# idonahum/photoVerse

Measured on AMD Instinct MI355X. Metric: denoising steps/sec at 512x512 bs=16, 50-step loop (2 UNet fwd + CFG + DPM-Solver++ step per step), higher is better.
Workload: dtype f16; 1 GPU; configs[1] shape timed over 96 steps instead of 50: SD-v1.5 UNet + PhotoVerse processors, 96-step loop, bs=16/GPU, 512x512 (64x64 latents), P=1, guidance 7.5, fp16; per_gpu_batch=16, global_batch=16, latent=64, parallelism=dp1 (batch-sharded, 1 all_gather), hip_graph=True, graph_branches=2

## Files before the change

### photoverse_amd/csrc/pv_gemm.hip

```cpp
#include "pv_gemm_dev.h"

namespace {

constexpr int BK = 64;
constexpr int ROW_BYTES = BK * 2;

template <int NF, int MIV = 4>
struct TileCfg {
    static constexpr int MI = MIV;
    static constexpr int BM = 2 * MI * 16;
    static constexpr int BN = NF * 32;
    static constexpr int NWAVES = 4;
    static constexpr int THREADS = NWAVES * 64;
    static constexpr int A_PER_WAVE = BM / 8 / NWAVES;
    static constexpr int STAGES = 2;
    static constexpr int A_BYTES = BM * ROW_BYTES;
    static constexpr int B_BYTES = BN * ROW_BYTES;
    static constexpr int STAGE_BYTES = A_BYTES + B_BYTES;
    static constexpr int SMEM_BYTES = STAGES * STAGE_BYTES;
    static constexpr int B_PIECES = NF * 4;
    static constexpr int B_PER_WAVE = (B_PIECES + NWAVES - 1) / NWAVES;
};

__device__ __forceinline__ float epi_act(float x, int act) {
    if (act == PV_ACT_SILU) return pv_silu(x);
    if (act == PV_ACT_QUICK_GELU) return pv_quick_gelu(x);
    if (act == PV_ACT_LEAKY_RELU) return x > 0.f ? x : 0.01f * x;
    return x;
}

__device__ __forceinline__ half8_t lds_frag(const char* base, int row, int chunk) {
    return *reinterpret_cast<const half8_t*>(base + row * ROW_BYTES + ((chunk ^ (row & 7)) << 4));
}

template <int N>
__device__ __forceinline__ void wait_vmcnt() {
    static_assert(N >= 0 && N < 64, "vmcnt is a 6-bit field");
    asm volatile("s_waitcnt vmcnt(%0)" ::"n"(N) : "memory");
}


__device__ __forceinline__ float row16_sum(float v) {
    v += __builtin_bit_cast(float, __builtin_amdgcn_update_dpp(0, __builtin_bit_cast(int, v), 0x128, 0xf, 0xf, false));
    v += __builtin_bit_cast(float, __builtin_amdgcn_update_dpp(0, __builtin_bit_cast(int, v), 0x124, 0xf, 0xf, false));
    v += __builtin_bit_cast(float, __builtin_amdgcn_update_dpp(0, __builtin_bit_cast(int, v), 0x122, 0xf, 0xf, false));
    v += __builtin_bit_cast(float, __builtin_amdgcn_update_dpp(0, __builtin_bit_cast(int, v), 0x121, 0xf, 0xf, false));
    return v;
}

template <int NF, bool CONV, bool GEGLU, bool CS = false, bool MULTI = false, int MIV = 4>
__global__ __launch_bounds__(256, MIV == 4 ? 2 : 3) void gemm_conv_kernel(const pv_gemm_params_dev p, const int tiles_n,
                                                                              const int nblk, const int order, const int tpw_arg) {
    const int tpw = MULTI ? tpw_arg : 1;
    using Cfg = TileCfg<NF, MIV>;
    static_assert(MIV == 4 || (!CS && !MULTI && !CONV), "the 64-row tile exists for plain Linear layers only");
    constexpr int BM = Cfg::BM;
    constexpr int NW = Cfg::NWAVES;
    constexpr int MI = Cfg::MI;
    constexpr int AP = Cfg::A_PER_WAVE;
    extern __shared__ __attribute__((aligned(16))) char smem[];

    const int lane = pv_lane_id();
    const int wave = pv_wave_id();
    const int bid = (order & 2) ? (int)blockIdx.x : pv_xcd_remap((int)blockIdx.x, nblk);
    const int m_fast = order & 1;
    const int tiles_m = nblk / tiles_n;
    const int tile_m = m_fast ? bid % tiles_m : bid / tiles_n;
    const int tile_n = (m_fast ? bid / tiles_m : bid % tiles_n) * tpw;
    const int m0 = tile_m * BM;
    int n0 = tile_n * Cfg::BN;

    const int cin = p.c0 + p.c1;
    const int K = p.taps * cin;
    const int nk_total = K / BK;
    const int nk_per = (nk_total + (int)gridDim.y - 1) / (int)gridDim.y;
    const int k_begin = (int)blockIdx.y * nk_per;
    const int nk = max(0, min(nk_total, k_begin + nk_per) - k_begin);

    const int lrow = lane >> 3;
    const int src_chunk = (lane & 7) ^ lrow;
    const int lane_cc2 = src_chunk * 16;
// ... 445 lines not shown
    if ((int)strlen(probe.name) >= name_len) return (int)hipErrorInvalidValue;
    strcpy(name, probe.name);
    if (workgroups) *workgroups = probe.wgs;
    return 0;
}

extern "C" int pv_gemm_conv(const pv_gemm_params* pp, void* stream_) {
    pv_gemm_params_dev p;
    static_cast<pv_gemm_params&>(p) = *pp;
    hipStream_t stream = reinterpret_cast<hipStream_t>(stream_);
    const int cin = p.c0 + p.c1;
    if (p.M <= 0 || p.N <= 0 || cin <= 0 || (cin % 64) || (p.c0 % 64) || (p.taps != 1 && p.taps != 9) || p.act == PV_ACT_GELU || p.splitk < 0 || p.splitk > 16 ||
        !p.a0 || !p.w || !p.out || (p.c1 && !p.a1) || p.hout * p.wout <= 0)
        return (int)hipErrorInvalidValue;
    if (p.colstats && (p.geglu || p.out_f32)) return (int)hipErrorInvalidValue;
    if (p.taps == 9 && !(p.pad == 1 || (p.pad == 0 && p.stride == 2 && !p.upsample))) return (int)hipErrorInvalidValue;
    {
        const size_t a_rows = p.taps == 9 ? (size_t)p.batch * p.hin * p.win : (size_t)p.M;
        const size_t b0 = ((a_rows - 1) * p.lda0 + p.c0) * 2, b1 = p.c1 ? ((a_rows - 1) * p.lda1 + p.c1) * 2 : 0;
        const size_t bw = (size_t)p.N * p.taps * cin * 2;
        if (b0 >= (1ull << 31) || b1 >= (1ull << 31) || bw >= (1ull << 31)) return (int)hipErrorInvalidValue;
        p.a0_bytes = (uint32_t)b0;
        p.a1_bytes = (uint32_t)b1;
        p.w_bytes = (uint32_t)bw;
    }
    if (p.geglu && (p.taps != 1 || (p.N % 128))) return (int)hipErrorInvalidValue;
    if (p.a_norm && (p.taps != 9 || (p.a_norm_act != PV_ACT_NONE && p.a_norm_act != PV_ACT_SILU))) return (int)hipErrorInvalidValue;
    {
        const int rc = pv_conv_big_launch(p, stream);
        if (rc >= 0) return rc;
        if (rc == -2 || p.a_norm) return (int)hipErrorInvalidValue;
    }
    if (p.ln_rowsum) return (int)hipErrorInvalidValue;
    if (p.geglu) return dispatch<4, false, true>(p, stream);
    const bool conv = p.taps == 9;
    if (p.N % 160 == 0) return conv ? dispatch<5, true, false>(p, stream) : dispatch<5, false, false>(p, stream);
    if (p.N % 128 == 0) return conv ? dispatch<4, true, false>(p, stream) : dispatch<4, false, false>(p, stream);
    return (int)hipErrorInvalidValue;
}
```

### photoverse_amd/csrc/pv_gemm_dev.h

```cpp
#pragma once
#include "pv_common.h"

struct pv_gemm_params_dev : pv_gemm_params {
    uint32_t a0_bytes, a1_bytes, w_bytes;
};

__attribute__((visibility("hidden"))) int pv_conv_big_launch(const pv_gemm_params_dev& p, hipStream_t stream);


__attribute__((visibility("hidden"))) int pv_gemm_splitk_reduce_launch(const pv_gemm_params_dev& p, int splits, hipStream_t stream);


struct pv_launch_probe {
    char name[160];
    long wgs;
};
extern thread_local pv_launch_probe* pv_gemm_probe;
```

### photoverse_amd/csrc/pv_rowgemm.hip

```cpp
#include "pv_common.h"
#include <stdlib.h>

namespace {

constexpr int RG_K = 320;
constexpr int RG_CHUNK = 160;
constexpr int RG_TILE = RG_CHUNK * 128;
constexpr int RG_SLOTS = 4;
constexpr int RG_SMEM = RG_SLOTS * RG_TILE;

struct pv_rowgemm_params_dev : pv_row_gemm_params {
    uint32_t w_bytes;
};

template <int N>
__device__ __forceinline__ void rg_wait_vmcnt() {
    static_assert(N >= 0 && N < 64, "vmcnt is a 6-bit field");
    asm volatile("s_waitcnt vmcnt(%0)" ::"n"(N) : "memory");
}

template <bool GEGLU>
__global__ __launch_bounds__(256, 2) void row_gemm_kernel(const pv_rowgemm_params_dev p) {
    constexpr int C = RG_K;
    constexpr int KK = C / 32;
    constexpr int KT = C / 64;
    constexpr int NFC = RG_CHUNK / 16;
    typedef unsigned uint4_t __attribute__((ext_vector_type(4)));
    typedef unsigned uint2_t __attribute__((ext_vector_type(2)));
    extern __shared__ __attribute__((aligned(16))) char smem[];

    const int lane = pv_lane_id(), wave = pv_wave_id();
    const int fr = lane & 15, g = lane >> 4;
    const int m0 = (int)blockIdx.x * 128;
    const int rows_here = min(128, p.M - m0);
    const int n_chunks = p.N / RG_CHUNK;
    const int NT = n_chunks * KT;

    const __amdgpu_buffer_rsrc_t rw = __builtin_amdgcn_make_buffer_rsrc(const_cast<void*>(p.w), 0, (int)p.w_bytes, 0x00020000);
    const __amdgpu_buffer_rsrc_t rx = __builtin_amdgcn_make_buffer_rsrc(const_cast<half_t*>(reinterpret_cast<const half_t*>(p.x)) + (size_t)m0 * p.ld_x, 0,
                                                                        rows_here * p.ld_x * 2, 0x00020000);
    const int ld_o = p.ld_out;
    const __amdgpu_buffer_rsrc_t ro = __builtin_amdgcn_make_buffer_rsrc(reinterpret_cast<half_t*>(p.out) + (size_t)m0 * ld_o, 0, rows_here * ld_o * 2, 0x00020000);

    const int lrow = lane >> 3;
    const unsigned w_lane_off = (unsigned)lrow * (unsigned)(C * 2) + (unsigned)(((lane & 7) ^ lrow) << 4);
    const unsigned piece_off = w_lane_off + (unsigned)(wave * 8) * (unsigned)(C * 2);
    auto issue_stage = [&](int t) {
        const int nc = t / KT, kt = t - nc * KT;
        char* dst = smem + (t & (RG_SLOTS - 1)) * RG_TILE;
        const int soff = nc * RG_CHUNK * (C * 2) + kt * 128;
#pragma unroll
        for (int i = 0; i < 5; ++i)
            __builtin_amdgcn_raw_ptr_buffer_load_lds(rw, PV_LDS_PTR(dst + (wave + 4 * i) * 1024), 16, (int)piece_off, soff + i * 32 * (C * 2), 0, 0);
    };
    auto wg_barrier = [&]() {
        asm volatile("s_waitcnt lgkmcnt(0)" ::: "memory");
        __builtin_amdgcn_s_barrier();
        asm volatile("" ::: "memory");
    };

    half8_t xf[KK][2];
    int mrow[2];
#pragma unroll
    for (int qi = 0; qi < 2; ++qi) {
        mrow[qi] = wave * 32 + qi * 16 + fr;
        const int off = mrow[qi] * p.ld_x * 2 + g * 16;
#pragma unroll
        for (int kk = 0; kk < KK; ++kk) xf[kk][qi] = __builtin_bit_cast(half8_t, __builtin_amdgcn_raw_buffer_load_b128(rx, off, kk * 64, 0));
    }
    issue_stage(0);
    issue_stage(1);
    if (p.x_norm) {
        const float* tab = p.x_norm + (size_t)(m0 / p.rows_per_image) * 2 * C + g * 8;
#pragma unroll
        for (int kk = 0; kk < KK; ++kk) {
            const float4_t s0 = *reinterpret_cast<const float4_t*>(tab + kk * 32), s1 = *reinterpret_cast<const float4_t*>(tab + kk * 32 + 4);
            const float4_t h0 = *reinterpret_cast<const float4_t*>(tab + C + kk * 32), h1 = *reinterpret_cast<const float4_t*>(tab + C + kk * 32 + 4);
#pragma unroll
            for (int qi = 0; qi < 2; ++qi)
#pragma unroll
                for (int j = 0; j < 8; ++j) xf[kk][qi][j] = (half_t)((float)xf[kk][qi][j] * (j < 4 ? s0[j & 3] : s1[j & 3]) + (j < 4 ? h0[j & 3] : h1[j & 3]));
        }
    }
    if (p.ln) {
        typedef _Float16 h2_t __attribute__((ext_vector_type(2)));
        const h2_t ones = h2_t{(half_t)1.0f, (half_t)1.0f};
#pragma unroll
        for (int qi = 0; qi < 2; ++qi) {
            float sum = 0.f;
#pragma unroll
            for (int kk = 0; kk < KK; ++kk)
#pragma unroll
                for (int j = 0; j < 4; ++j) sum = __builtin_amdgcn_fdot2(h2_t{xf[kk][qi][2 * j], xf[kk][qi][2 * j + 1]}, ones, sum, false);
            const float mean = pv_quad_sum(sum) * (1.0f / (float)C);
            const half_t mh = (half_t)mean;
            const h2_t nm = h2_t{(half_t)(-mh), (half_t)(-mh)};
            float sq = 0.f;
#pragma unroll
            for (int kk = 0; kk < KK; ++kk)
#pragma unroll
                for (int j = 0; j < 4; ++j) {
                    const h2_t d = h2_t{xf[kk][qi][2 * j], xf[kk][qi][2 * j + 1]} + nm;
                    sq = __builtin_amdgcn_fdot2(d, d, sq, false);
                }
            const float dm = mean - (float)mh;
            const float var = pv_quad_sum(sq) * (1.0f / (float)C) - dm * dm;
            const float rstd = rsqrtf(fmaxf(var, 0.f) + p.ln_eps);
            const float nmr = -mean * rstd;
#pragma unroll
            for (int kk = 0; kk < KK; ++kk)
#pragma unroll
                for (int j = 0; j < 8; ++j) xf[kk][qi][j] = (half_t)fmaf((float)xf[kk][qi][j], rstd, nmr);
        }
    }
    rg_wait_vmcnt<0>();

    const int ring_lane[2] = {fr * 128 + ((g ^ (fr & 7)) << 4), fr * 128 + (((4 + g) ^ (fr & 7)) << 4)};
    const int pcol = (g & 1) ? 16 + (g - 1) * 4 : g * 4;
    constexpr int OUT_PER_CHUNK = GEGLU ? RG_CHUNK / 2 : RG_CHUNK;
    constexpr int STORES = GEGLU ? 6 : 10;

    float4_t acc[NFC][2];
    for (int it = 0; it < n_chunks / 2; ++it) {
        const int t0 = it * (2 * KT);
#pragma unroll
        for (int j = 0; j < 2 * KT; ++j) {
            const int t = t0 + j;
            const int kt = j % KT;
            const int nc = 2 * it + j / KT;
            if ((j & 1) == 0) {
                const bool stores_since = (j == 6) || (j == 0 && it > 0);
                if (t >= 2) {
                    if (stores_since) rg_wait_vmcnt<STORES>(); else rg_wait_vmcnt<0>();
                }
                wg_barrier();
                if (t + 2 < NT) issue_stage(t + 2);
                if (t + 3 < NT) issue_stage(t + 3);
            }
            if (kt == 0) {
#pragma unroll
                for (int i = 0; i < NFC; ++i)
                    acc[i][0] = acc[i][1] = p.bias ? *reinterpret_cast<const float4_t*>(p.bias + nc * RG_CHUNK + i * 16 + g * 4) : float4_t{0.f, 0.f, 0.f, 0.f};
            }
            const char* slot = smem + (t & (RG_SLOTS - 1)) * RG_TILE;
#pragma unroll
            for (int ks = 0; ks < 2; ++ks) {
                const char* base = slot + ring_lane[ks];
#pragma unroll
                for (int i = 0; i < NFC; ++i) {
                    const half8_t a = *reinterpret_cast<const half8_t*>(base + i * 2048);
#pragma unroll
                    for (int qi = 0; qi < 2; ++qi) acc[i][qi] = __builtin_amdgcn_mfma_f32_16x16x32_f16(a, xf[2 * kt + ks][qi], acc[i][qi], 0, 0, 0);
                }
            }
            if (kt == KT - 1) {
                const int ocol0 = nc * OUT_PER_CHUNK;
#pragma unroll
                for (int qi = 0; qi < 2; ++qi) {
                    const int ooff = mrow[qi] * ld_o * 2 + ocol0 * 2;
                    unsigned pk[GEGLU ? NFC / 2 : NFC][2];
                    if (GEGLU) {
#pragma unroll
                        for (int q = 0; q < NFC / 2; ++q) {
                            const float4_t v = acc[2 * q][qi], gt = acc[2 * q + 1][qi];
                            pk[q][0] = __builtin_bit_cast(unsigned, half2_t{(half_t)(v[0] * pv_gelu_erf(gt[0])), (half_t)(v[1] * pv_gelu_erf(gt[1]))});
                            pk[q][1] = __builtin_bit_cast(unsigned, half2_t{(half_t)(v[2] * pv_gelu_erf(gt[2])), (half_t)(v[3] * pv_gelu_erf(gt[3]))});
                        }
                    } else {
#pragma unroll
                        for (int i = 0; i < NFC; ++i) {
                            const float4_t v = acc[i][qi];
                            pk[i][0] = __builtin_bit_cast(unsigned, half2_t{(half_t)v[0], (half_t)v[1]});
                            pk[i][1] = __builtin_bit_cast(unsigned, half2_t{(half_t)v[2], (half_t)v[3]});
                        }
                    }
                    constexpr int NOUT = GEGLU ? NFC / 2 : NFC;
#pragma unroll
                    for (int q = 0; q < NOUT / 2; ++q) {
                        const auto v0 = __builtin_amdgcn_permlane16_swap(pk[2 * q][0], pk[2 * q + 1][0], false, false);
                        const auto v1 = __builtin_amdgcn_permlane16_swap(pk[2 * q][1], pk[2 * q + 1][1], false, false);
                        const unsigned sa0 = v0[0], sb0 = v0[1], sa1 = v1[0], sb1 = v1[1];
                        __builtin_amdgcn_raw_buffer_store_b128(uint4_t{sa0, sa1, sb0, sb1}, ro, ooff + pcol * 2 + q * 64, 0, 0);
                        asm volatile("s_nop 1" ::: "memory");
                    }
                    if (NOUT & 1)
                        __builtin_amdgcn_raw_buffer_store_b64(uint2_t{pk[NOUT - 1][0], pk[NOUT - 1][1]}, ro, ooff + g * 8 + (NOUT - 1) * 32, 0, 0);
                }
                __builtin_amdgcn_sched_barrier(0);
            }
        }
    }
}

}

extern "C" int pv_row_gemm(const pv_row_gemm_params* pp, void* stream) {
    pv_rowgemm_params_dev p;
    static_cast<pv_row_gemm_params&>(p) = *pp;
    if (!p.x || !p.w || !p.out || p.M <= 0 || p.K != RG_K || p.N <= 0 || (p.N % (2 * RG_CHUNK)) || (p.ld_x % 8) || (p.ld_out % 8) || p.ld_x < RG_K ||
        p.ld_out < (p.geglu ? p.N / 2 : p.N) || (p.x_norm && (p.ln || p.rows_per_image <= 0 || (p.rows_per_image % 128) || (p.M % p.rows_per_image))))
        return (int)hipErrorInvalidValue;
    if ((size_t)p.N * RG_K * 2 >= (1ull << 31)) return (int)hipErrorInvalidValue;
    p.w_bytes = (uint32_t)p.N * RG_K * 2;
    static bool attr_set_dev[64][2] = {};
    int dev_id = 0;
    (void)hipGetDevice(&dev_id);
    bool& attr_set = attr_set_dev[dev_id & 63][p.geglu ? 1 : 0];
    auto kern = p.geglu ? row_gemm_kernel<true> : row_gemm_kernel<false>;
    if (!attr_set) {
        hipError_t e = hipFuncSetAttribute(reinterpret_cast<const void*>(kern), hipFuncAttributeMaxDynamicSharedMemorySize, RG_SMEM);
        if (e != hipSuccess) return (int)e;
        attr_set = true;
    }
    hipLaunchKernelGGL(kern, dim3((unsigned)((p.M + 127) / 128)), dim3(256), RG_SMEM, (hipStream_t)stream, p);
    return PV_CHECK_LAUNCH();
}
```

### photoverse_amd/build.py

```python
from __future__ import annotations

import concurrent.futures as cf
import os
import shutil
import subprocess
import sys

HERE = os.path.dirname(os.path.abspath(__file__))
CSRC = os.path.join(HERE, "csrc")
LIBDIR = os.path.join(HERE, "lib")
LIB = os.path.join(LIBDIR, "libphotoverse_hip.so")
SOURCES = ["pv_gemm.hip", "pv_convbig.hip", "pv_norm.hip", "pv_attn.hip", "pv_misc.hip", "pv_xfused.hip", "pv_xq.hip", "pv_rowgemm.hip", "pv_backward.hip", "pv_train.hip", "pv_attnbwd.hip"]
FLAGS = ["--offload-arch=gfx950", "-O3", "-std=c++17", "-fPIC"]
EXTRA_FLAGS = {"pv_attn.hip": ["-mllvm", "-amdgpu-mfma-vgpr-form", "-fno-honor-nans"],
               "pv_xfused.hip": ["-mllvm", "-amdgpu-mfma-vgpr-form", "-fno-honor-nans",
                                 "-mllvm", "-pragma-unroll-threshold=4000000"],

               "pv_xq.hip": ["-mllvm", "-amdgpu-mfma-vgpr-form", "-fno-honor-nans"],
               "pv_rowgemm.hip": ["-mllvm", "-amdgpu-mfma-vgpr-form"],
               "pv_train.hip": ["-mllvm", "-amdgpu-mfma-vgpr-form", "-fno-honor-nans"],
               "pv_attnbwd.hip": ["-mllvm", "-amdgpu-mfma-vgpr-form", "-fno-honor-nans"]}


def _hipcc() -> str:
    exe = shutil.which("hipcc") or "/opt/rocm/bin/hipcc"
    if not os.path.exists(exe):
        raise RuntimeError("hipcc not found: the HIP extension cannot be built")
    return exe


def _stale(out: str, deps) -> bool:
    if not os.path.exists(out):
        return True
    t = os.path.getmtime(out)
    return any(os.path.getmtime(d) > t for d in deps)


def build_lib(force: bool = False, verbose: bool = True) -> str:
    os.makedirs(LIBDIR, exist_ok=True)
    hipcc = _hipcc()
    headers = [os.path.join(CSRC, "pv_common.h"), os.path.join(CSRC, "pv_gemm_dev.h"), os.path.join(os.path.dirname(HERE), "include", "photoverse_hip.h"), __file__]
    objs, jobs = [], []
    for src in SOURCES:
        s = os.path.join(CSRC, src)
        o = os.path.join(LIBDIR, src.replace(".hip", ".o"))
        objs.append(o)
        if force or _stale(o, [s] + headers):
            jobs.append([hipcc, *FLAGS, *EXTRA_FLAGS.get(src, []), "-c", s, "-o", o])
    if jobs:
        with cf.ThreadPoolExecutor(max_workers=4) as ex:
            for cmd, res in zip(jobs, ex.map(lambda c: subprocess.run(c, capture_output=True, text=True), jobs)):
                if res.returncode != 0:
# ... 15 lines not shown
```

Baseline: 33.93 denoising steps/s (bs=16 per GPU, summed over GPUs).

## Add weight-streaming K=320 GEMM kernel with fused bias, residual and colstats

Adds a specialized kernel for 320x320 linear layers with residual (e.g. attention output projections at the 64x64 level). Each block keeps its 128 activation rows in registers and streams the weights through an LDS ring, writing both 160-wide output chunks. Bias and residual adds are fused, with optional column statistics computed from LDS. It is dispatched ahead of the generic tiled GEMM when M is large, so it adds a new hand-scheduled code path with its own correctness risk.

```diff
diff --git a/photoverse_amd/csrc/pv_gemm.hip b/photoverse_amd/csrc/pv_gemm.hip
--- a/photoverse_amd/csrc/pv_gemm.hip
+++ b/photoverse_amd/csrc/pv_gemm.hip
@@ -39,14 +39,6 @@
     asm volatile("s_waitcnt vmcnt(%0)" ::"n"(N) : "memory");
 }
 
-
-__device__ __forceinline__ float row16_sum(float v) {
-    v += __builtin_bit_cast(float, __builtin_amdgcn_update_dpp(0, __builtin_bit_cast(int, v), 0x128, 0xf, 0xf, false));
-    v += __builtin_bit_cast(float, __builtin_amdgcn_update_dpp(0, __builtin_bit_cast(int, v), 0x124, 0xf, 0xf, false));
-    v += __builtin_bit_cast(float, __builtin_amdgcn_update_dpp(0, __builtin_bit_cast(int, v), 0x122, 0xf, 0xf, false));
-    v += __builtin_bit_cast(float, __builtin_amdgcn_update_dpp(0, __builtin_bit_cast(int, v), 0x121, 0xf, 0xf, false));
-    return v;
-}
 
 template <int NF, bool CONV, bool GEGLU, bool CS = false, bool MULTI = false, int MIV = 4>
 __global__ __launch_bounds__(256, MIV == 4 ? 2 : 3) void gemm_conv_kernel(const pv_gemm_params_dev p, const int tiles_n,
@@ -560,6 +552,10 @@
     if (p.ln_rowsum) return (int)hipErrorInvalidValue;
     if (p.geglu) return dispatch<4, false, true>(p, stream);
     const bool conv = p.taps == 9;
+    {
+        const int rc = pv_k320_stream_launch(p, stream);
+        if (rc >= 0) return rc;
+    }
     if (p.N % 160 == 0) return conv ? dispatch<5, true, false>(p, stream) : dispatch<5, false, false>(p, stream);
     if (p.N % 128 == 0) return conv ? dispatch<4, true, false>(p, stream) : dispatch<4, false, false>(p, stream);
     return (int)hipErrorInvalidValue;
diff --git a/photoverse_amd/csrc/pv_gemm_dev.h b/photoverse_amd/csrc/pv_gemm_dev.h
--- a/photoverse_amd/csrc/pv_gemm_dev.h
+++ b/photoverse_amd/csrc/pv_gemm_dev.h
@@ -8,6 +8,9 @@
 __attribute__((visibility("hidden"))) int pv_conv_big_launch(const pv_gemm_params_dev& p, hipStream_t stream);
 
 
+__attribute__((visibility("hidden"))) int pv_k320_stream_launch(const pv_gemm_params_dev& p, hipStream_t stream);
+
+
 __attribute__((visibility("hidden"))) int pv_gemm_splitk_reduce_launch(const pv_gemm_params_dev& p, int splits, hipStream_t stream);
 
 
@@ -16,3 +19,11 @@
     long wgs;
 };
 extern thread_local pv_launch_probe* pv_gemm_probe;
+
+__device__ __forceinline__ float row16_sum(float v) {
+    v += __builtin_bit_cast(float, __builtin_amdgcn_update_dpp(0, __builtin_bit_cast(int, v), 0x128, 0xf, 0xf, false));
+    v += __builtin_bit_cast(float, __builtin_amdgcn_update_dpp(0, __builtin_bit_cast(int, v), 0x124, 0xf, 0xf, false));
+    v += __builtin_bit_cast(float, __builtin_amdgcn_update_dpp(0, __builtin_bit_cast(int, v), 0x122, 0xf, 0xf, false));
+    v += __builtin_bit_cast(float, __builtin_amdgcn_update_dpp(0, __builtin_bit_cast(int, v), 0x121, 0xf, 0xf, false));
+    return v;
+}
diff --git a/photoverse_amd/csrc/pv_rowgemm.hip b/photoverse_amd/csrc/pv_rowgemm.hip
--- a/photoverse_amd/csrc/pv_rowgemm.hip
+++ b/photoverse_amd/csrc/pv_rowgemm.hip
@@ -1,4 +1,4 @@
-#include "pv_common.h"
+#include "pv_gemm_dev.h"
 #include <stdlib.h>
 
 namespace {
@@ -17,6 +17,29 @@
 __device__ __forceinline__ void rg_wait_vmcnt() {
     static_assert(N >= 0 && N < 64, "vmcnt is a 6-bit field");
     asm volatile("s_waitcnt vmcnt(%0)" ::"n"(N) : "memory");
+}
+
+__device__ __forceinline__ float4_t bias_frag(const float4_t v, const int i) {
+    float4_t r;
+#pragma unroll
+    for (int c = 0; c < 4; ++c) {
+        const int x = __builtin_bit_cast(int, (float)v[c]);
+        int y = 0;
+        switch (i) {
+            case 0: y = __builtin_amdgcn_update_dpp(0, x, 0x150, 0xf, 0xf, false); break;
+            case 1: y = __builtin_amdgcn_update_dpp(0, x, 0x151, 0xf, 0xf, false); break;
+            case 2: y = __builtin_amdgcn_update_dpp(0, x, 0x152, 0xf, 0xf, false); break;
+            case 3: y = __builtin_amdgcn_update_dpp(0, x, 0x153, 0xf, 0xf, false); break;
+            case 4: y = __builtin_amdgcn_update_dpp(0, x, 0x154, 0xf, 0xf, false); break;
+            case 5: y = __builtin_amdgcn_update_dpp(0, x, 0x155, 0xf, 0xf, false); break;
+            case 6: y = __builtin_amdgcn_update_dpp(0, x, 0x156, 0xf, 0xf, false); break;
+            case 7: y = __builtin_amdgcn_update_dpp(0, x, 0x157, 0xf, 0xf, false); break;
+            case 8: y = __builtin_amdgcn_update_dpp(0, x, 0x158, 0xf, 0xf, false); break;
+            default: y = __builtin_amdgcn_update_dpp(0, x, 0x159, 0xf, 0xf, false); break;
+        }
+        r[c] = __builtin_bit_cast(float, y);
+    }
+    return r;
 }
 
 template <bool GEGLU>
@@ -192,6 +215,224 @@
     }
 }
 
+template <bool CS>
+__global__ __launch_bounds__(256, 2) void k320_stream_kernel(const pv_gemm_params_dev p) {
+    constexpr int C = RG_K;
+    constexpr int KK = C / 32;
+    constexpr int KT = C / 64;
+    constexpr int NFC = RG_CHUNK / 16;
+    constexpr int NT = 2 * KT;
+    constexpr int STORES = NFC;
+    constexpr int RES = NFC;
+    constexpr int BACK = 10;
+    typedef unsigned uint4_t __attribute__((ext_vector_type(4)));
+    typedef unsigned uint2_t __attribute__((ext_vector_type(2)));
+    extern __shared__ __attribute__((aligned(16))) char smem[];
+
+    const int lane = pv_lane_id(), wave = pv_wave_id();
+    const int fr = lane & 15, g = lane >> 4;
+    const int m0 = (int)blockIdx.x * 128;
+    const int rows_here = min(128, p.M - m0);
+
+    const __amdgpu_buffer_rsrc_t rw = __builtin_amdgcn_make_buffer_rsrc(const_cast<void*>(p.w), 0, (int)p.w_bytes, 0x00020000);
+    const __amdgpu_buffer_rsrc_t rx = __builtin_amdgcn_make_buffer_rsrc(const_cast<half_t*>(reinterpret_cast<const half_t*>(p.a0)) + (size_t)m0 * p.lda0, 0,
+                                                                        rows_here * p.lda0 * 2, 0x00020000);
+    const __amdgpu_buffer_rsrc_t rr = __builtin_amdgcn_make_buffer_rsrc(const_cast<half_t*>(reinterpret_cast<const half_t*>(p.residual)) + (size_t)m0 * p.ldr, 0,
+                                                                        rows_here * p.ldr * 2, 0x00020000);
+    const __amdgpu_buffer_rsrc_t ro = __builtin_amdgcn_make_buffer_rsrc(reinterpret_cast<half_t*>(p.out) + (size_t)m0 * p.ldc, 0, rows_here * p.ldc * 2, 0x00020000);
+
+    const int lrow = lane >> 3;
+    const unsigned piece_off = (unsigned)(wave * 8 + lrow) * (unsigned)(C * 2) + (unsigned)(((lane & 7) ^ lrow) << 4);
+    auto issue_stage = [&](int t) {
+        const int nc = t / KT, kt = t - nc * KT;
+        char* dst = smem + (t & (RG_SLOTS - 1)) * RG_TILE;
+        const int soff = nc * RG_CHUNK * (C * 2) + kt * 128;
+#pragma unroll
+        for (int i = 0; i < 5; ++i)
+            __builtin_amdgcn_raw_ptr_buffer_load_lds(rw, PV_LDS_PTR(dst + (wave + 4 * i) * 1024), 16, (int)piece_off, soff + i * 32 * (C * 2), 0, 0);
+    };
+    auto wg_barrier = [&]() {
+        asm volatile("s_waitcnt lgkmcnt(0)" ::: "memory");
+        __builtin_amdgcn_s_barrier();
+        asm volatile("" ::: "memory");
+    };
+
+    const int pcol = (g & 1) ? 16 + (g - 1) * 4 : g * 4;
+    constexpr int CS_GROUP = 20 * 256;
+    const int cs_lane = (g >> 1) * 256 + fr * 16 + (g & 1) * 8;
+    half8_t xf[KK][2];
+    int mrow[2];
+    uint4_t res[NFC / 2][2];
+    auto load_res = [&](int nc) {
+#pragma unroll
+        for (int qi = 0; qi < 2; ++qi)
+#pragma unroll
+            for (int q = 0; q < NFC / 2; ++q)
+                res[q][qi] = __builtin_amdgcn_raw_buffer_load_b128(rr, mrow[qi] * p.ldr * 2 + pcol * 2 + (nc * (RG_CHUNK * 2) + q * 64), 0, 0);
+    };
+#pragma unroll
+    for (int qi = 0; qi < 2; ++qi) {
+        mrow[qi] = wave * 32 + qi * 16 + fr;
+        const int off = mrow[qi] * p.lda0 * 2 + g * 16;
+#pragma unroll
+        for (int kk = 0; kk < KK; ++kk) xf[kk][qi] = __builtin_bit_cast(half8_t, __builtin_amdgcn_raw_buffer_load_b128(rx, off, kk * 64, 0));
+    }
+    issue_stage(0);
+    issue_stage(1);
+    load_res(0);
+    auto load_bias = [&](int nc) {
+        return p.bias ? *reinterpret_cast<const float4_t*>(p.bias + nc * RG_CHUNK + min(fr, NFC - 1) * 16 + g * 4) : float4_t{0.f, 0.f, 0.f, 0.f};
+    };
+    float4_t bv = load_bias(0);
+    rg_wait_vmcnt<0>();
+
+    const int ring_lane[2] = {fr * 128 + ((g ^ (fr & 7)) << 4), fr * 128 + (((4 + g) ^ (fr & 7)) << 4)};
+    float4_t acc[NFC][2];
+#pragma unroll
+    for (int j = 0; j < NT; ++j) {
+        const int kt = j % KT, nc = j / KT;
+        if ((j & 1) == 0) {
+            if (j >= 2) {
+                if (j == 6) rg_wait_vmcnt<STORES + RES>(); else rg_wait_vmcnt<0>();
+            }
+            wg_barrier();
+            if (j + 2 < NT) issue_stage(j + 2);
+            if (j + 3 < NT) issue_stage(j + 3);
+            if (CS && j == NT - 2) {
+#pragma unroll
+                for (int i = 0; i < BACK; ++i) {
+                    const int k = wave + 4 * i, grp = k / 5, t = k - grp * 5;
+                    __builtin_amdgcn_raw_ptr_buffer_load_lds(ro, PV_LDS_PTR(smem + 2 * RG_TILE + k * 1024), 16, (grp * 16 + fr) * p.ldc * 2 + g * 16 + t * 64, 0, 0, 0);
+                }
+            }
+        }
+        if (kt == 0) {
+#pragma unroll
+            for (int i = 0; i < NFC; ++i) acc[i][0] = acc[i][1] = float4_t{0.f, 0.f, 0.f, 0.f};
+        }
+        const char* slot = smem + (j & (RG_SLOTS - 1)) * RG_TILE;
+#pragma unroll
+        for (int ks = 0; ks < 2; ++ks) {
+            const char* base = slot + ring_lane[ks];
+#pragma unroll
+            for (int i = 0; i < NFC; ++i) {
+                const half8_t a = *reinterpret_cast<const half8_t*>(base + i * 2048);
+#pragma unroll
+                for (int qi = 0; qi < 2; ++qi) acc[i][qi] = __builtin_amdgcn_mfma_f32_16x16x32_f16(a, xf[2 * kt + ks][qi], acc[i][qi], 0, 0, 0);
+            }
+        }
+        if (kt == KT - 1) {
+            if (CS && nc == 1) wg_barrier();
+            __builtin_amdgcn_sched_barrier(0);
+#pragma unroll
+            for (int q = 0; q < NFC / 2; ++q) {
+                const float4_t b0 = bias_frag(bv, 2 * q), b1 = bias_frag(bv, 2 * q + 1);
+#pragma unroll
+                for (int qi = 0; qi < 2; ++qi) {
+                    const auto u0 = __builtin_amdgcn_permlane16_swap(res[q][qi][0], res[q][qi][2], false, false);
+                    const auto u1 = __builtin_amdgcn_permlane16_swap(res[q][qi][1], res[q][qi][3], false, false);
+                    const unsigned ra0 = u0[0], rb0 = u0[1], ra1 = u1[0], rb1 = u1[1];
+                    const half2_t r00 = __builtin_bit_cast(half2_t, ra0), r01 = __builtin_bit_cast(half2_t, ra1);
+                    const half2_t r10 = __builtin_bit_cast(half2_t, rb0), r11 = __builtin_bit_cast(half2_t, rb1);
+                    float4_t v0 = acc[2 * q][qi] + b0, v1 = acc[2 * q + 1][qi] + b1;
+                    v0[0] += (float)r00[0]; v0[1] += (float)r00[1]; v0[2] += (float)r01[0]; v0[3] += (float)r01[1];
+                    v1[0] += (float)r10[0]; v1[1] += (float)r10[1]; v1[2] += (float)r11[0]; v1[3] += (float)r11[1];
+                    const unsigned p00 = __builtin_bit_cast(unsigned, half2_t{(half_t)v0[0], (half_t)v0[1]}), p01 = __builtin_bit_cast(unsigned, half2_t{(half_t)v0[2], (half_t)v0[3]});
+                    const unsigned p10 = __builtin_bit_cast(unsigned, half2_t{(half_t)v1[0], (half_t)v1[1]}), p11 = __builtin_bit_cast(unsigned, half2_t{(half_t)v1[2], (half_t)v1[3]});
+                    if (CS && nc == 1) {
+                        *reinterpret_cast<uint2_t*>(smem + (wave * 2 + qi) * CS_GROUP + (2 * q) * 512 + cs_lane) = uint2_t{p00, p01};
+                        *reinterpret_cast<uint2_t*>(smem + (wave * 2 + qi) * CS_GROUP + (2 * q + 1) * 512 + cs_lane) = uint2_t{p10, p11};
+                    }
+                    const auto s0 = __builtin_amdgcn_permlane16_swap(p00, p10, false, false);
+                    const auto s1 = __builtin_amdgcn_permlane16_swap(p01, p11, false, false);
+                    const unsigned sa0 = s0[0], sb0 = s0[1], sa1 = s1[0], sb1 = s1[1];
+                    __builtin_amdgcn_raw_buffer_store_b128(uint4_t{sa0, sa1, sb0, sb1}, ro, mrow[qi] * p.ldc * 2 + pcol * 2 + (nc * (RG_CHUNK * 2) + q * 64), 0, 0);
+                    asm volatile("s_nop 1" ::: "memory");
+                }
+            }
+            __builtin_amdgcn_sched_barrier(0);
+            if (nc == 0) {
+                load_res(1);
+                bv = load_bias(1);
+                __builtin_amdgcn_sched_barrier(0);
+            }
+        }
+    }
+    if (CS) {
+        rg_wait_vmcnt<STORES>();
+        wg_barrier();
+        const int blk = wave >> 1, nc = wave & 1;
+        if (m0 + blk * 64 >= p.M) return;
+        const char* src = smem + (nc == 0 ? 2 * RG_TILE : 0) + blk * 4 * CS_GROUP + cs_lane;
+        float4_t cs[NFC], cq[NFC];
+#pragma unroll
+        for (int i = 0; i < NFC; ++i) cs[i] = cq[i] = float4_t{0.f, 0.f, 0.f, 0.f};
+#pragma unroll
+        for (int mi = 0; mi < 4; ++mi) {
+            if (m0 + blk * 64 + mi * 16 + fr < p.M) {
+#pragma unroll
+                for (int i = 0; i < NFC; ++i) {
+                    const half4_t h = *reinterpret_cast<const half4_t*>(src + mi * CS_GROUP + i * 512);
+#pragma unroll
+                    for (int r = 0; r < 4; ++r) {
+                        const float f = (float)h[r];
+                        cs[i][r] += f;
+                        cq[i][r] += f * f;
+                    }
+                }
+            }
+        }
+#pragma unroll
+        for (int i = 0; i < NFC; ++i)
+#pragma unroll
+            for (int r = 0; r < 4; ++r) {
+                cs[i][r] = row16_sum(cs[i][r]);
+                cq[i][r] = row16_sum(cq[i][r]);
+            }
+        if (fr == 0) {
+            float* dst = p.colstats + ((size_t)(m0 / 64 + blk) * 2) * p.N + nc * RG_CHUNK + g * 4;
+#pragma unroll
+            for (int i = 0; i < NFC; ++i) {
+                *reinterpret_cast<float4_t*>(dst + i * 16) = cs[i];
+                *reinterpret_cast<float4_t*>(dst + p.N + i * 16) = cq[i];
+            }
+        }
+    }
+}
+
+}
+
+int pv_k320_stream_launch(const pv_gemm_params_dev& p, hipStream_t stream) {
+    const char* sw = getenv("PV_K320_STREAM");
+    const int mode = sw ? atoi(sw) : 1;
+    if (mode == 0 || (mode == 2 && p.colstats)) return -1;
+    const char* env = getenv("PV_CONV_BIG");
+    const int min_tiles = p.big_tile_min ? p.big_tile_min : (env ? atoi(env) : 256);
+    if (min_tiles <= 0) return -1;
+    if (p.taps != 1 || p.c1 || p.c0 != RG_K || p.N != 2 * RG_CHUNK || p.out_f32 || p.geglu || (p.splitk > 1 && p.splitk_ws) || p.ln_rowsum || p.a_norm || p.rowadd ||
+        p.act != PV_ACT_NONE || !p.residual)
+        return -1;
+    if ((p.lda0 % 8) || (p.ldr % 8) || (p.ldc % 8) || p.lda0 < RG_K || p.ldr < p.N || p.ldc < p.N) return -1;
+    const long tiles = ((long)p.M + 127) / 128;
+    if (tiles < 2L * min_tiles) return -1;
+    const bool cs = p.colstats != nullptr;
+    if (pv_gemm_probe) {
+        snprintf(pv_gemm_probe->name, sizeof(pv_gemm_probe->name), "k320_stream_kernel<%s>", cs ? "true" : "false");
+        pv_gemm_probe->wgs = tiles;
+        return 0;
+    }
+    static bool attr_set_dev[64][2] = {};
+    int dev_id = 0;
+    (void)hipGetDevice(&dev_id);
+    bool& attr_set = attr_set_dev[dev_id & 63][cs ? 1 : 0];
+    auto kern = cs ? k320_stream_kernel<true> : k320_stream_kernel<false>;
+    if (!attr_set) {
+        hipError_t e = hipFuncSetAttribute(reinterpret_cast<const void*>(kern), hipFuncAttributeMaxDynamicSharedMemorySize, RG_SMEM);
+        if (e != hipSuccess) return (int)e;
+        attr_set = true;
+    }
+    hipLaunchKernelGGL(kern, dim3((unsigned)tiles), dim3(256), RG_SMEM, stream, p);
+    return PV_CHECK_LAUNCH();
 }
 
 extern "C" int pv_row_gemm(const pv_row_gemm_params* pp, void* stream) {
```

Result: no change. 34.11 denoising steps/s (bs=16 per GPU, summed over GPUs), median of 6 (+0.5%).

## Add row-GEMM kernel with fused bias+residual epilogue for K=320,N=320 GEMMs

Applied to the files above, without the earlier changes.

Adds a specialised row-GEMM kernel for the K=320, N=320 1x1 projections that carry a residual, with large M (at least 32768 rows). It keeps the activation rows in registers, streams the weight chunks through an LDS ring, and fuses the bias and residual add into the store epilogue. The general GEMM dispatcher tries this path first, and the file is now built with a high unroll threshold. The aim is to replace the generic tiled GEMM for the 64x64-resolution attention projections (proj_out, to_out) with a kernel that has more weight reuse. The risk is extra register pressure and more code paths to validate.

```diff
diff --git a/photoverse_amd/build.py b/photoverse_amd/build.py
--- a/photoverse_amd/build.py
+++ b/photoverse_amd/build.py
@@ -17,7 +17,8 @@
                                  "-mllvm", "-pragma-unroll-threshold=4000000"],
 
                "pv_xq.hip": ["-mllvm", "-amdgpu-mfma-vgpr-form", "-fno-honor-nans"],
-               "pv_rowgemm.hip": ["-mllvm", "-amdgpu-mfma-vgpr-form"],
+               "pv_rowgemm.hip": ["-mllvm", "-amdgpu-mfma-vgpr-form",
+                                  "-mllvm", "-pragma-unroll-threshold=4000000"],
                "pv_train.hip": ["-mllvm", "-amdgpu-mfma-vgpr-form", "-fno-honor-nans"],
                "pv_attnbwd.hip": ["-mllvm", "-amdgpu-mfma-vgpr-form", "-fno-honor-nans"]}
 
diff --git a/photoverse_amd/csrc/pv_gemm.hip b/photoverse_amd/csrc/pv_gemm.hip
--- a/photoverse_amd/csrc/pv_gemm.hip
+++ b/photoverse_amd/csrc/pv_gemm.hip
@@ -558,6 +558,10 @@
         if (rc == -2 || p.a_norm) return (int)hipErrorInvalidValue;
     }
     if (p.ln_rowsum) return (int)hipErrorInvalidValue;
+    {
+        const int rc = pv_row_gemm_res_launch(p, stream);
+        if (rc >= 0) return rc;
+    }
     if (p.geglu) return dispatch<4, false, true>(p, stream);
     const bool conv = p.taps == 9;
     if (p.N % 160 == 0) return conv ? dispatch<5, true, false>(p, stream) : dispatch<5, false, false>(p, stream);
diff --git a/photoverse_amd/csrc/pv_gemm_dev.h b/photoverse_amd/csrc/pv_gemm_dev.h
--- a/photoverse_amd/csrc/pv_gemm_dev.h
+++ b/photoverse_amd/csrc/pv_gemm_dev.h
@@ -8,6 +8,9 @@
 __attribute__((visibility("hidden"))) int pv_conv_big_launch(const pv_gemm_params_dev& p, hipStream_t stream);
 
 
+__attribute__((visibility("hidden"))) int pv_row_gemm_res_launch(const pv_gemm_params_dev& p, hipStream_t stream);
+
+
 __attribute__((visibility("hidden"))) int pv_gemm_splitk_reduce_launch(const pv_gemm_params_dev& p, int splits, hipStream_t stream);
 
 
diff --git a/photoverse_amd/csrc/pv_rowgemm.hip b/photoverse_amd/csrc/pv_rowgemm.hip
--- a/photoverse_amd/csrc/pv_rowgemm.hip
+++ b/photoverse_amd/csrc/pv_rowgemm.hip
@@ -1,4 +1,5 @@
-#include "pv_common.h"
+#include "pv_gemm_dev.h"
+#include <stdio.h>
 #include <stdlib.h>
 
 namespace {
@@ -192,6 +193,189 @@
     }
 }
 
+struct pv_rowgemm_res_params {
+    const void* x; const void* w; const void* residual; void* out;
+    const float* bias;
+    int32_t ld_x, ld_res, ld_out, M;
+    uint32_t w_bytes;
+};
+
+__global__ __launch_bounds__(256, 2) void row_gemm_res_kernel(const pv_rowgemm_res_params p) {
+    constexpr int C = RG_K;
+    constexpr int KK = C / 32;
+    constexpr int KT = C / 64;
+    constexpr int NFC = RG_CHUNK / 16;
+    constexpr int NT = 2 * KT;
+    typedef unsigned uint4_t __attribute__((ext_vector_type(4)));
+    extern __shared__ __attribute__((aligned(16))) char smem[];
+
+    const int lane = pv_lane_id(), wave = pv_wave_id();
+    const int fr = lane & 15, g = lane >> 4;
+    const int m0 = (int)blockIdx.x * 128;
+    const int rows_here = min(128, p.M - m0);
+    const int ld_o = p.ld_out, ld_r = p.ld_res;
+
+    const __amdgpu_buffer_rsrc_t rw = __builtin_amdgcn_make_buffer_rsrc(const_cast<void*>(p.w), 0, (int)p.w_bytes, 0x00020000);
+    const __amdgpu_buffer_rsrc_t rx = __builtin_amdgcn_make_buffer_rsrc(const_cast<half_t*>(reinterpret_cast<const half_t*>(p.x)) + (size_t)m0 * p.ld_x, 0,
+                                                                        rows_here * p.ld_x * 2, 0x00020000);
+    const __amdgpu_buffer_rsrc_t rr = __builtin_amdgcn_make_buffer_rsrc(const_cast<half_t*>(reinterpret_cast<const half_t*>(p.residual)) + (size_t)m0 * ld_r, 0,
+                                                                        rows_here * ld_r * 2, 0x00020000);
+    const __amdgpu_buffer_rsrc_t ro = __builtin_amdgcn_make_buffer_rsrc(reinterpret_cast<half_t*>(p.out) + (size_t)m0 * ld_o, 0, rows_here * ld_o * 2, 0x00020000);
+    const __amdgpu_buffer_rsrc_t rb = __builtin_amdgcn_make_buffer_rsrc(const_cast<float*>(p.bias), 0, p.bias ? 2 * RG_CHUNK * 4 : 0, 0x00020000);
+
+    const int lrow = lane >> 3;
+    const unsigned w_lane_off = (unsigned)lrow * (unsigned)(C * 2) + (unsigned)(((lane & 7) ^ lrow) << 4);
+    const unsigned piece_off = w_lane_off + (unsigned)(wave * 8) * (unsigned)(C * 2);
+    auto issue_stage = [&](int t) {
+        const int nc = t / KT, kt = t - nc * KT;
+        char* dst = smem + (t & (RG_SLOTS - 1)) * RG_TILE;
+        const int soff = nc * RG_CHUNK * (C * 2) + kt * 128;
+#pragma unroll
+        for (int i = 0; i < 5; ++i)
+            __builtin_amdgcn_raw_ptr_buffer_load_lds(rw, PV_LDS_PTR(dst + (wave + 4 * i) * 1024), 16, (int)piece_off, soff + i * 32 * (C * 2), 0, 0);
+    };
+    auto wg_barrier = [&]() {
+        asm volatile("s_waitcnt lgkmcnt(0)" ::: "memory");
+        __builtin_amdgcn_s_barrier();
+        asm volatile("" ::: "memory");
+    };
+
+    const int pcol = (g & 1) ? 16 + (g - 1) * 4 : g * 4;
+    half8_t xf[KK][2];
+    int mrow[2];
+    uint4_t rs[2][NFC / 2];
+    constexpr int RES_LOADS = NFC / 2;
+    auto load_residual = [&](int nc, int qi) {
+        __builtin_amdgcn_sched_barrier(0);
+#pragma unroll
+        for (int q = 0; q < NFC / 2; ++q)
+            rs[qi][q] = __builtin_amdgcn_raw_buffer_load_b128(rr, mrow[qi] * ld_r * 2 + nc * (RG_CHUNK * 2) + pcol * 2 + q * 64, 0, 0);
+        __builtin_amdgcn_sched_barrier(0);
+    };
+#pragma unroll
+    for (int qi = 0; qi < 2; ++qi) {
+        mrow[qi] = wave * 32 + qi * 16 + fr;
+        const int off = mrow[qi] * p.ld_x * 2 + g * 16;
+#pragma unroll
+        for (int kk = 0; kk < KK; ++kk) xf[kk][qi] = __builtin_bit_cast(half8_t, __builtin_amdgcn_raw_buffer_load_b128(rx, off, kk * 64, 0));
+    }
+    load_residual(0, 0);
+    float bl[2 * RG_CHUNK / 64];
+#pragma unroll
+    for (int j = 0; j < 2 * RG_CHUNK / 64; ++j) bl[j] = __builtin_bit_cast(float, __builtin_amdgcn_raw_buffer_load_b32(rb, (64 * j + lane) * 4, 0, 0));
+    issue_stage(0);
+    issue_stage(1);
+    rg_wait_vmcnt<0>();
+
+    const int ring_lane[2] = {fr * 128 + ((g ^ (fr & 7)) << 4), fr * 128 + (((4 + g) ^ (fr & 7)) << 4)};
+    constexpr int STORES = NFC;
+
+    float4_t acc[NFC][2];
+#pragma unroll
+    for (int t = 0; t < NT; ++t) {
+        const int kt = t % KT, nc = t / KT;
+        if ((t & 1) == 0) {
+            if (t == 6) rg_wait_vmcnt<STORES + RES_LOADS>(); else if (t >= 2) rg_wait_vmcnt<0>();
+            wg_barrier();
+            if (t + 2 < NT) issue_stage(t + 2);
+            if (t + 3 < NT) issue_stage(t + 3);
+        }
+        if (kt == KT - 1) load_residual(nc, 1);
+        if (kt == 0) {
+#pragma unroll
+            for (int i = 0; i < NFC; ++i) acc[i][0] = acc[i][1] = float4_t{0.f, 0.f, 0.f, 0.f};
+        }
+        const char* slot = smem + (t & (RG_SLOTS - 1)) * RG_TILE;
+#pragma unroll
+        for (int ks = 0; ks < 2; ++ks) {
+            const char* base = slot + ring_lane[ks];
+#pragma unroll
+            for (int i = 0; i < NFC; ++i) {
+                const half8_t a = *reinterpret_cast<const half8_t*>(base + i * 2048);
+#pragma unroll
+                for (int qi = 0; qi < 2; ++qi) acc[i][qi] = __builtin_amdgcn_mfma_f32_16x16x32_f16(a, xf[2 * kt + ks][qi], acc[i][qi], 0, 0, 0);
+            }
+        }
+        if (kt == KT - 1) {
+#pragma unroll
+            for (int qi = 0; qi < 2; ++qi) {
+                const int ooff = mrow[qi] * ld_o * 2 + nc * (RG_CHUNK * 2);
+                unsigned pk[NFC][2];
+#pragma unroll
+                for (int q = 0; q < NFC / 2; ++q) {
+                    const uint4_t r = rs[qi][q];
+                    const auto u0 = __builtin_amdgcn_permlane16_swap(r[0], r[2], false, false);
+                    const auto u1 = __builtin_amdgcn_permlane16_swap(r[1], r[3], false, false);
+                    const half2_t res[2][2] = {{__builtin_bit_cast(half2_t, (unsigned)u0[0]), __builtin_bit_cast(half2_t, (unsigned)u1[0])},
+                                               {__builtin_bit_cast(half2_t, (unsigned)u0[1]), __builtin_bit_cast(half2_t, (unsigned)u1[1])}};
+#pragma unroll
+                    for (int h = 0; h < 2; ++h) {
+                        const int i = 2 * q + h;
+                        const int e0 = nc * RG_CHUNK + i * 16;
+                        float4_t b;
+#pragma unroll
+                        for (int r = 0; r < 4; ++r)
+                            b[r] = __builtin_bit_cast(float, __builtin_amdgcn_ds_bpermute((e0 % 64 + g * 4 + r) * 4, __builtin_bit_cast(int, bl[e0 / 64])));
+                        float4_t v = acc[i][qi] + b;
+                        v += float4_t{(float)res[h][0][0], (float)res[h][0][1], (float)res[h][1][0], (float)res[h][1][1]};
+                        pk[i][0] = __builtin_bit_cast(unsigned, half2_t{(half_t)v[0], (half_t)v[1]});
+                        pk[i][1] = __builtin_bit_cast(unsigned, half2_t{(half_t)v[2], (half_t)v[3]});
+                    }
+                }
+#pragma unroll
+                for (int q = 0; q < NFC / 2; ++q) {
+                    const auto v0 = __builtin_amdgcn_permlane16_swap(pk[2 * q][0], pk[2 * q + 1][0], false, false);
+                    const auto v1 = __builtin_amdgcn_permlane16_swap(pk[2 * q][1], pk[2 * q + 1][1], false, false);
+                    const unsigned sa0 = v0[0], sb0 = v0[1], sa1 = v1[0], sb1 = v1[1];
+                    __builtin_amdgcn_raw_buffer_store_b128(uint4_t{sa0, sa1, sb0, sb1}, ro, ooff + pcol * 2 + q * 64, 0, 0);
+                    asm volatile("s_nop 1" ::: "memory");
+                }
+            }
+            if (nc == 0) load_residual(1, 0);
+            __builtin_amdgcn_sched_barrier(0);
+        }
+    }
+}
+
+constexpr int RG_RES_MIN_ROWS = 256 * 128;
+
+}
+
+int pv_row_gemm_res_launch(const pv_gemm_params_dev& g, hipStream_t stream) {
+    if (g.taps != 1 || g.c0 != RG_K || g.c1 != 0 || g.N != 2 * RG_CHUNK || !g.residual || g.act != PV_ACT_NONE || g.out_f32 || g.geglu ||
+        (g.splitk > 1 && g.splitk_ws) || g.rowadd || g.ln_rowsum || g.a_norm || g.colstats || g.M < RG_RES_MIN_ROWS)
+        return -1;
+    if ((g.lda0 % 8) || (g.ldr % 8) || (g.ldc % 8) || g.lda0 < RG_K || g.ldr < g.N || g.ldc < g.N ||
+        (((uintptr_t)g.a0 | (uintptr_t)g.residual | (uintptr_t)g.out | (uintptr_t)g.w | (uintptr_t)g.bias) & 15))
+        return -1;
+    const unsigned wgs = (unsigned)((g.M + 127) / 128);
+    if (pv_gemm_probe) {
+        snprintf(pv_gemm_probe->name, sizeof(pv_gemm_probe->name), "row_gemm_res_kernel");
+        pv_gemm_probe->wgs = (long)wgs;
+        return 0;
+    }
+    pv_rowgemm_res_params p;
+    p.x = g.a0;
+    p.w = g.w;
+    p.residual = g.residual;
+    p.out = g.out;
+    p.bias = g.bias;
+    p.ld_x = g.lda0;
+    p.ld_res = g.ldr;
+    p.ld_out = g.ldc;
+    p.M = g.M;
+    p.w_bytes = g.w_bytes;
+    static bool attr_set_dev[64] = {};
+    int dev_id = 0;
+    (void)hipGetDevice(&dev_id);
+    bool& attr_set = attr_set_dev[dev_id & 63];
+    if (!attr_set) {
+        hipError_t e = hipFuncSetAttribute(reinterpret_cast<const void*>(row_gemm_res_kernel), hipFuncAttributeMaxDynamicSharedMemorySize, RG_SMEM);
+        if (e != hipSuccess) return (int)e;
+        attr_set = true;
+    }
+    hipLaunchKernelGGL(row_gemm_res_kernel, dim3(wgs), dim3(256), RG_SMEM, stream, p);
+    return PV_CHECK_LAUNCH();
 }
 
 extern "C" int pv_row_gemm(const pv_row_gemm_params* pp, void* stream) {
```

New measurement: 33.39 denoising steps/s (bs=16 per GPU, summed over GPUs) before, 33.56 denoising steps/s (bs=16 per GPU, summed over GPUs) after, median of 6. No clear change (+0.5%).

## Restructure row GEMM into 32-column full-K stages with software-pipelined epilogue

Applied to the files above, without the earlier changes.

Changes the weight staging from 160-column chunks split along K into 32-output-column stages that each hold the full K=320 slice. Accumulation then runs over ping-pong accumulator sets, and the previous stage's GEGLU/convert/store epilogue is interleaved with the current stage's MFMAs. Bias is prefetched through buffer loads alongside the LDS stages, and LDS fragment reads are software-pipelined three deep. The goal is to hide the epilogue (erf GELU, permlane swaps, stores) and the bias loads behind matrix work and to cut accumulator register pressure. The cost is more barriers per column, more complex vmcnt accounting, and a risk of wrong counts in the waits.

```diff
diff --git a/photoverse_amd/csrc/pv_rowgemm.hip b/photoverse_amd/csrc/pv_rowgemm.hip
--- a/photoverse_amd/csrc/pv_rowgemm.hip
+++ b/photoverse_amd/csrc/pv_rowgemm.hip
@@ -5,7 +5,8 @@
 
 constexpr int RG_K = 320;
 constexpr int RG_CHUNK = 160;
-constexpr int RG_TILE = RG_CHUNK * 128;
+constexpr int RG_STAGE = 32;
+constexpr int RG_TILE = RG_STAGE * RG_K * 2;
 constexpr int RG_SLOTS = 4;
 constexpr int RG_SMEM = RG_SLOTS * RG_TILE;
 
@@ -24,17 +25,14 @@
     constexpr int C = RG_K;
     constexpr int KK = C / 32;
     constexpr int KT = C / 64;
-    constexpr int NFC = RG_CHUNK / 16;
     typedef unsigned uint4_t __attribute__((ext_vector_type(4)));
-    typedef unsigned uint2_t __attribute__((ext_vector_type(2)));
     extern __shared__ __attribute__((aligned(16))) char smem[];
 
     const int lane = pv_lane_id(), wave = pv_wave_id();
     const int fr = lane & 15, g = lane >> 4;
     const int m0 = (int)blockIdx.x * 128;
     const int rows_here = min(128, p.M - m0);
-    const int n_chunks = p.N / RG_CHUNK;
-    const int NT = n_chunks * KT;
+    const int NT = p.N / RG_STAGE;
 
     const __amdgpu_buffer_rsrc_t rw = __builtin_amdgcn_make_buffer_rsrc(const_cast<void*>(p.w), 0, (int)p.w_bytes, 0x00020000);
     const __amdgpu_buffer_rsrc_t rx = __builtin_amdgcn_make_buffer_rsrc(const_cast<half_t*>(reinterpret_cast<const half_t*>(p.x)) + (size_t)m0 * p.ld_x, 0,
@@ -46,12 +44,16 @@
     const unsigned w_lane_off = (unsigned)lrow * (unsigned)(C * 2) + (unsigned)(((lane & 7) ^ lrow) << 4);
     const unsigned piece_off = w_lane_off + (unsigned)(wave * 8) * (unsigned)(C * 2);
     auto issue_stage = [&](int t) {
-        const int nc = t / KT, kt = t - nc * KT;
         char* dst = smem + (t & (RG_SLOTS - 1)) * RG_TILE;
-        const int soff = nc * RG_CHUNK * (C * 2) + kt * 128;
-#pragma unroll
-        for (int i = 0; i < 5; ++i)
-            __builtin_amdgcn_raw_ptr_buffer_load_lds(rw, PV_LDS_PTR(dst + (wave + 4 * i) * 1024), 16, (int)piece_off, soff + i * 32 * (C * 2), 0, 0);
+        const int soff = min(t, NT - 1) * RG_TILE;
+#pragma unroll
+        for (int i = 0; i < KT; ++i)
+            __builtin_amdgcn_raw_ptr_buffer_load_lds(rw, PV_LDS_PTR(dst + i * 4096 + wave * 1024), 16, (int)piece_off, soff + i * 128, 0, 0);
+    };
+    const __amdgpu_buffer_rsrc_t rb = __builtin_amdgcn_make_buffer_rsrc(const_cast<void*>(p.bias ? (const void*)p.bias : p.w), 0, p.bias ? p.N * 4 : 0, 0x00020000);
+    auto load_bias = [&](int t, float4_t (&b)[2]) {
+#pragma unroll
+        for (int f = 0; f < 2; ++f) b[f] = __builtin_bit_cast(float4_t, __builtin_amdgcn_raw_buffer_load_b128(rb, g * 16, min(t, NT - 1) * (RG_STAGE * 4) + f * 64, 0));
     };
     auto wg_barrier = [&]() {
         asm volatile("s_waitcnt lgkmcnt(0)" ::: "memory");
@@ -70,6 +72,9 @@
     }
     issue_stage(0);
     issue_stage(1);
+    float4_t bia[2][2];
+    load_bias(0, bia[0]);
+    load_bias(1, bia[1]);
     if (p.x_norm) {
         const float* tab = p.x_norm + (size_t)(m0 / p.rows_per_image) * 2 * C + g * 8;
 #pragma unroll
@@ -117,79 +122,102 @@
 
     const int ring_lane[2] = {fr * 128 + ((g ^ (fr & 7)) << 4), fr * 128 + (((4 + g) ^ (fr & 7)) << 4)};
     const int pcol = (g & 1) ? 16 + (g - 1) * 4 : g * 4;
-    constexpr int OUT_PER_CHUNK = GEGLU ? RG_CHUNK / 2 : RG_CHUNK;
-    constexpr int STORES = GEGLU ? 6 : 10;
-
-    float4_t acc[NFC][2];
-    for (int it = 0; it < n_chunks / 2; ++it) {
-        const int t0 = it * (2 * KT);
-#pragma unroll
-        for (int j = 0; j < 2 * KT; ++j) {
-            const int t = t0 + j;
-            const int kt = j % KT;
-            const int nc = 2 * it + j / KT;
-            if ((j & 1) == 0) {
-                const bool stores_since = (j == 6) || (j == 0 && it > 0);
-                if (t >= 2) {
-                    if (stores_since) rg_wait_vmcnt<STORES>(); else rg_wait_vmcnt<0>();
-                }
-                wg_barrier();
-                if (t + 2 < NT) issue_stage(t + 2);
-                if (t + 3 < NT) issue_stage(t + 3);
-            }
-            if (kt == 0) {
-#pragma unroll
-                for (int i = 0; i < NFC; ++i)
-                    acc[i][0] = acc[i][1] = p.bias ? *reinterpret_cast<const float4_t*>(p.bias + nc * RG_CHUNK + i * 16 + g * 4) : float4_t{0.f, 0.f, 0.f, 0.f};
-            }
-            const char* slot = smem + (t & (RG_SLOTS - 1)) * RG_TILE;
-#pragma unroll
-            for (int ks = 0; ks < 2; ++ks) {
-                const char* base = slot + ring_lane[ks];
-#pragma unroll
-                for (int i = 0; i < NFC; ++i) {
-                    const half8_t a = *reinterpret_cast<const half8_t*>(base + i * 2048);
-#pragma unroll
-                    for (int qi = 0; qi < 2; ++qi) acc[i][qi] = __builtin_amdgcn_mfma_f32_16x16x32_f16(a, xf[2 * kt + ks][qi], acc[i][qi], 0, 0, 0);
+    const int ovo[2] = {mrow[0] * ld_o * 2 + pcol * 2, mrow[1] * ld_o * 2 + pcol * 2};
+    constexpr int S_EVEN = GEGLU ? 0 : 2, S_ODD = 2;
+
+    float4_t acc[2][2][2];
+    float gl[2][4];
+    unsigned held[2][2];
+
+    auto epilogue = [&](int s, const float4_t (&E)[2][2], const bool odd, const int kk) {
+        if (GEGLU) {
+            if (kk % 5 != 4) {
+                const int qi = kk / 5, j = kk % 5;
+                float x = E[1][qi][j];
+                asm volatile("" : "+v"(x));
+                float r = E[0][qi][j] * pv_gelu_erf(x);
+                asm volatile("" : "+v"(r));
+                gl[qi][j] = r;
+            } else {
+                const int qi = kk / 5;
+                const unsigned p0 = __builtin_bit_cast(unsigned, half2_t{(half_t)gl[qi][0], (half_t)gl[qi][1]});
+                const unsigned p1 = __builtin_bit_cast(unsigned, half2_t{(half_t)gl[qi][2], (half_t)gl[qi][3]});
+                if (!odd) {
+                    held[qi][0] = p0;
+                    held[qi][1] = p1;
+                    asm volatile("" : "+v"(held[qi][0]), "+v"(held[qi][1]));
+                } else {
+                    const auto v0 = __builtin_amdgcn_permlane16_swap(held[qi][0], p0, false, false);
+                    const auto v1 = __builtin_amdgcn_permlane16_swap(held[qi][1], p1, false, false);
+                    __builtin_amdgcn_raw_buffer_store_b128(uint4_t{v0[0], v1[0], v0[1], v1[1]}, ro, ovo[qi] + (s >> 1) * 64, 0, 0);
+                    asm volatile("s_nop 1" ::: "memory");
                 }
             }
-            if (kt == KT - 1) {
-                const int ocol0 = nc * OUT_PER_CHUNK;
-#pragma unroll
-                for (int qi = 0; qi < 2; ++qi) {
-                    const int ooff = mrow[qi] * ld_o * 2 + ocol0 * 2;
-                    unsigned pk[GEGLU ? NFC / 2 : NFC][2];
-                    if (GEGLU) {
-#pragma unroll
-                        for (int q = 0; q < NFC / 2; ++q) {
-                            const float4_t v = acc[2 * q][qi], gt = acc[2 * q + 1][qi];
-                            pk[q][0] = __builtin_bit_cast(unsigned, half2_t{(half_t)(v[0] * pv_gelu_erf(gt[0])), (half_t)(v[1] * pv_gelu_erf(gt[1]))});
-                            pk[q][1] = __builtin_bit_cast(unsigned, half2_t{(half_t)(v[2] * pv_gelu_erf(gt[2])), (half_t)(v[3] * pv_gelu_erf(gt[3]))});
-                        }
-                    } else {
-#pragma unroll
-                        for (int i = 0; i < NFC; ++i) {
-                            const float4_t v = acc[i][qi];
-                            pk[i][0] = __builtin_bit_cast(unsigned, half2_t{(half_t)v[0], (half_t)v[1]});
-                            pk[i][1] = __builtin_bit_cast(unsigned, half2_t{(half_t)v[2], (half_t)v[3]});
-                        }
-                    }
-                    constexpr int NOUT = GEGLU ? NFC / 2 : NFC;
-#pragma unroll
-                    for (int q = 0; q < NOUT / 2; ++q) {
-                        const auto v0 = __builtin_amdgcn_permlane16_swap(pk[2 * q][0], pk[2 * q + 1][0], false, false);
-                        const auto v1 = __builtin_amdgcn_permlane16_swap(pk[2 * q][1], pk[2 * q + 1][1], false, false);
-                        const unsigned sa0 = v0[0], sb0 = v0[1], sa1 = v1[0], sb1 = v1[1];
-                        __builtin_amdgcn_raw_buffer_store_b128(uint4_t{sa0, sa1, sb0, sb1}, ro, ooff + pcol * 2 + q * 64, 0, 0);
-                        asm volatile("s_nop 1" ::: "memory");
-                    }
-                    if (NOUT & 1)
-                        __builtin_amdgcn_raw_buffer_store_b64(uint2_t{pk[NOUT - 1][0], pk[NOUT - 1][1]}, ro, ooff + g * 8 + (NOUT - 1) * 32, 0, 0);
-                }
-                __builtin_amdgcn_sched_barrier(0);
+        } else if (kk == 2 || kk == 6) {
+            const int qi = kk >> 2;
+            unsigned pk[2][2];
+#pragma unroll
+            for (int f = 0; f < 2; ++f) {
+                const float4_t v = E[f][qi];
+                pk[f][0] = __builtin_bit_cast(unsigned, half2_t{(half_t)v[0], (half_t)v[1]});
+                pk[f][1] = __builtin_bit_cast(unsigned, half2_t{(half_t)v[2], (half_t)v[3]});
             }
-        }
-    }
+            const auto v0 = __builtin_amdgcn_permlane16_swap(pk[0][0], pk[1][0], false, false);
+            const auto v1 = __builtin_amdgcn_permlane16_swap(pk[0][1], pk[1][1], false, false);
+            __builtin_amdgcn_raw_buffer_store_b128(uint4_t{v0[0], v1[0], v0[1], v1[1]}, ro, ovo[qi] + s * 64, 0, 0);
+            asm volatile("s_nop 1" ::: "memory");
+        }
+    };
+    auto stage = [&](int t, float4_t (&A)[2][2], const float4_t (&b)[2], const float4_t (&E)[2][2], const bool drain) {
+        const bool odd = (&A == &acc[1]);
+#pragma unroll
+        for (int f = 0; f < 2; ++f) A[f][0] = A[f][1] = b[f];
+        const char* slot = smem + (t & (RG_SLOTS - 1)) * RG_TILE;
+        half8_t a[3][2];
+#pragma unroll
+        for (int kk = 0; kk < 2; ++kk)
+#pragma unroll
+            for (int f = 0; f < 2; ++f) a[kk][f] = *reinterpret_cast<const half8_t*>(slot + (kk >> 1) * 4096 + f * 2048 + ring_lane[kk & 1]);
+#pragma unroll
+        for (int kk = 0; kk < KK; ++kk) {
+            if (kk + 2 < KK) {
+#pragma unroll
+                for (int f = 0; f < 2; ++f)
+                    a[(kk + 2) % 3][f] = *reinterpret_cast<const half8_t*>(slot + ((kk + 2) >> 1) * 4096 + f * 2048 + ring_lane[kk & 1]);
+            }
+#pragma unroll
+            for (int f = 0; f < 2; ++f)
+#pragma unroll
+                for (int qi = 0; qi < 2; ++qi) A[f][qi] = __builtin_amdgcn_mfma_f32_16x16x32_f16(a[kk % 3][f], xf[kk][qi], A[f][qi], 0, 0, 0);
+            if (drain) epilogue(t - 1, E, !odd, kk);
+            __builtin_amdgcn_sched_barrier(0);
+        }
+    };
+
+    for (int u = 0; u < NT / 2; ++u) {
+        const int t = 2 * u;
+        if (u == 1) rg_wait_vmcnt<S_EVEN>();
+        else if (u > 1) rg_wait_vmcnt<S_ODD + S_EVEN>();
+        wg_barrier();
+        float4_t bnext[2][2];
+        load_bias(t + 2, bnext[0]);
+        load_bias(t + 3, bnext[1]);
+        asm volatile("" ::: "memory");
+        issue_stage(t + 2);
+        issue_stage(t + 3);
+        asm volatile("" ::: "memory");
+        __builtin_amdgcn_sched_barrier(0);
+        if (u == 0) stage(t, acc[0], bia[0], acc[1], false);
+        else stage(t, acc[0], bia[0], acc[1], true);
+        stage(t + 1, acc[1], bia[1], acc[0], true);
+#pragma unroll
+        for (int f = 0; f < 2; ++f) {
+            bia[0][f] = bnext[0][f];
+            bia[1][f] = bnext[1][f];
+        }
+    }
+#pragma unroll
+    for (int kk = 0; kk < KK; ++kk) epilogue(NT - 1, acc[1], true, kk);
 }
 
 }
```

Measured after the change: 32.47 denoising steps/s (bs=16 per GPU, summed over GPUs) before, 32.68 denoising steps/s (bs=16 per GPU, summed over GPUs) after, median of 6. Within noise of the previous version (+0.6%).
